# getterupper/PreWorld

Hardware: AMD Instinct MI355X
Metric: samples/sec (6-cam frame -> 200x200x16 occ) (higher is better)
Workload: dtype f32 as hi+lo f16 (3 MFMA per product block, f32 accumulate)

## Files before the change

preworld_amd/csrc/pw_forecast.hip:

```cpp
#include "pw_h2.h"

typedef float f32x16 __attribute__((ext_vector_type(16)));

namespace {
constexpr int C = 32;
constexpr int HID = 128;
constexpr int W1P = 4 * 4 * 64 * 4;
constexpr int W2P = 4 * 4 * 64 * 4;
}

__device__ __forceinline__ int row_of(int r, int h) { return (r & 3) + 8 * (r >> 2) + 4 * h; }

__device__ __forceinline__ float softplus_t20(float x) {
  const float t = __builtin_amdgcn_exp2f(-fabsf(x) * 1.44269504088896341f);
  return fmaf(__builtin_amdgcn_logf(1.f + t), 0.693147180559945309f, fmaxf(x, 0.f));
}

__global__ void __launch_bounds__(256)
k_forecast_prologue(const float* __restrict__ ego, int ego_dim, const float* __restrict__ w0,
                    const float* __restrict__ b0, const float* __restrict__ w2,
                    const float* __restrict__ b2, const float* __restrict__ w4,
                    const float* __restrict__ b4, const float* __restrict__ fw1,
                    const float* __restrict__ fb1, float* __restrict__ ego_feat,
                    float* __restrict__ c1, float* __restrict__ c1p) {
  __shared__ float h1[256], h2[256], e[C];
  const int t = threadIdx.x, s = blockIdx.x;
  const float* x = ego + (size_t)s * ego_dim;
  float acc = b0[t];
  for (int i = 0; i < ego_dim; ++i) acc += x[i] * w0[t * ego_dim + i];
  h1[t] = fmaxf(acc, 0.f);
  __syncthreads();
  acc = b2[t];
  for (int i = 0; i < 256; ++i) acc += h1[i] * w2[t * 256 + i];
  h2[t] = fmaxf(acc, 0.f);
  __syncthreads();
  if (t < C) {
    acc = b4[t];
    for (int i = 0; i < 256; ++i) acc += h2[i] * w4[t * 256 + i];
    e[t] = acc;
    ego_feat[(size_t)s * C + t] = acc;
  }
  __syncthreads();
  if (t < HID) {
    acc = fb1[t];
    for (int i = 0; i < C; ++i) acc += e[i] * fw1[t * 2 * C + C + i];
    c1[(size_t)s * HID + t] = acc;
    const int tile = t >> 5, row = t & 31;
    const int h = (row >> 2) & 1, r = (row & 3) + 4 * (row >> 3);
    c1p[(size_t)s * HID + h * 64 + tile * 16 + r] = acc;
  }
}

__global__ void k_forecast_pack(const float* __restrict__ fw1, const float* __restrict__ fw2,
                                float* __restrict__ w1p, float* __restrict__ w2p) {
  int idx = blockIdx.x * blockDim.x + threadIdx.x;
  if (idx >= W1P) return;
  int e = idx & 3, lane = (idx >> 2) & 63, q = (idx >> 8) & 3, t = idx >> 10;
  int i = lane & 31, h = lane >> 5;
  int k = row_of(4 * q + e, h);
  w1p[idx] = fw1[(size_t)(t * 32 + i) * (2 * C) + k];
  w2p[idx] = fw2[(size_t)i * HID + t * 32 + k];
}

__global__ void __launch_bounds__(256, 4)
k_forecast(const float* __restrict__ v0, long long n_vox_per_sample, int n_samples,
           const float* __restrict__ w1p, const float* __restrict__ w2p,
           const float* __restrict__ c1p, const float* __restrict__ fb2, int n_steps,
           float* __restrict__ states ) {
  extern __shared__ __attribute__((aligned(16))) float lds[];
  float* l_w1 = lds;
  float* l_w2 = lds + W1P;
  const int tid = threadIdx.x, lane = tid & 63, wave = tid >> 6;
  const int h = lane >> 5, j = lane & 31;
  for (int k = tid; k < W1P / 4; k += 256) {
    reinterpret_cast<float4*>(l_w1)[k] = reinterpret_cast<const float4*>(w1p)[k];
    reinterpret_cast<float4*>(l_w2)[k] = reinterpret_cast<const float4*>(w2p)[k];
  }
  __syncthreads();

  const long long n_total = n_vox_per_sample * n_samples;
  const long long n_tiles = (n_total + 31) / 32;
  float b2r[16];
#pragma unroll
  for (int s = 0; s < 16; ++s) b2r[s] = fb2[row_of(s, h)];

  for (long long tile = (long long)blockIdx.x * 4 + wave; tile < n_tiles;
       tile += (long long)gridDim.x * 4) {
    const long long m0 = tile * 32;
    long long m = m0 + j;
    const bool valid = m < n_total;
    if (!valid) m = n_total - 1;
    const int sample = (int)(m / n_vox_per_sample);
    const float* c1s = c1p + (size_t)sample * HID + h * 64;
    float v[16];
    const float* src = v0 + (size_t)m * C + 4 * h;
#pragma unroll
    for (int q = 0; q < 4; ++q) {
      float4 t4 = *reinterpret_cast<const float4*>(src + 8 * q);
      v[4 * q + 0] = t4.x; v[4 * q + 1] = t4.y; v[4 * q + 2] = t4.z; v[4 * q + 3] = t4.w;
    }
    for (int step = 0; step < n_steps; ++step) {
      f32x16 o;
#pragma unroll
      for (int s = 0; s < 16; ++s) o[s] = b2r[s];
#pragma unroll 1
      for (int t = 0; t < 4; ++t) {
        f32x16 hid;
#pragma unroll
        for (int q = 0; q < 4; ++q) {
          const float4 c4 = *reinterpret_cast<const float4*>(c1s + t * 16 + q * 4);
          hid[4 * q + 0] = c4.x; hid[4 * q + 1] = c4.y; hid[4 * q + 2] = c4.z; hid[4 * q + 3] = c4.w;
        }
#pragma unroll
        for (int sq = 0; sq < 4; ++sq) {
          const float4 a4 = *reinterpret_cast<const float4*>(l_w1 + ((t * 4 + sq) * 64 + lane) * 4);
          const float av[4] = {a4.x, a4.y, a4.z, a4.w};
#pragma unroll
          for (int e = 0; e < 4; ++e)
            hid = __builtin_amdgcn_mfma_f32_32x32x2f32(av[e], v[4 * sq + e], hid, 0, 0, 0);
        }
#pragma unroll
        for (int r = 0; r < 16; ++r) hid[r] = softplus_t20(hid[r]);
#pragma unroll
        for (int rq = 0; rq < 4; ++rq) {
          const float4 a4 = *reinterpret_cast<const float4*>(l_w2 + ((t * 4 + rq) * 64 + lane) * 4);
          const float av[4] = {a4.x, a4.y, a4.z, a4.w};
#pragma unroll
          for (int e = 0; e < 4; ++e)
            o = __builtin_amdgcn_mfma_f32_32x32x2f32(av[e], hid[4 * rq + e], o, 0, 0, 0);
        }
      }
#pragma unroll
      for (int s = 0; s < 16; ++s) v[s] = o[s] + v[s];
      if (valid) {
        float* dst = states + ((size_t)step * n_total + m) * C + 4 * h;
#pragma unroll
        for (int q = 0; q < 4; ++q)
          *reinterpret_cast<float4*>(dst + 8 * q) =
              make_float4(v[4 * q + 0], v[4 * q + 1], v[4 * q + 2], v[4 * q + 3]);
      }
    }
  }
}

PW_API int pw_forecast_pack(const float* fusion_w1, const float* fusion_w2, float* w1p, float* w2p,
                            void* stream) {
  PW_CHECK_ARG(fusion_w1 && fusion_w2 && w1p && w2p, "pw_forecast_pack: null pointer");
  hipLaunchKernelGGL(k_forecast_pack, dim3(W1P / 256), dim3(256), 0, pw_stream(stream), fusion_w1,
                     fusion_w2, w1p, w2p);
  PW_CHECK_LAUNCH();
  return PW_OK;
}

PW_API int pw_forecast_prologue(const float* ego, int n_samples, int ego_dim, const float* plan_w0,
                                const float* plan_b0, const float* plan_w2, const float* plan_b2,
                                const float* plan_w4, const float* plan_b4, const float* fusion_w1,
                                const float* fusion_b1, float* ego_feat, float* c1, float* c1p,
                                void* stream) {
  PW_CHECK_ARG(ego && plan_w0 && plan_b0 && plan_w2 && plan_b2 && plan_w4 && plan_b4 && fusion_w1 &&
                   fusion_b1 && ego_feat && c1 && c1p,
               "pw_forecast_prologue: null pointer");
  PW_CHECK_ARG(n_samples > 0 && ego_dim > 0, "pw_forecast_prologue: bad sizes");
  hipLaunchKernelGGL(k_forecast_prologue, dim3(n_samples), dim3(256), 0, pw_stream(stream), ego,
                     ego_dim, plan_w0, plan_b0, plan_w2, plan_b2, plan_w4, plan_b4, fusion_w1,
                     fusion_b1, ego_feat, c1, c1p);
  PW_CHECK_LAUNCH();
  return PW_OK;
}

PW_API int pw_forecast_steps(const float* v0, int64_t n_vox_per_sample, int n_samples,
                             const float* w1p, const float* w2p, const float* c1p,
                             const float* fusion_b2, int n_steps, float* states, void* stream) {
  PW_CHECK_ARG(v0 && w1p && w2p && c1p && fusion_b2 && states, "pw_forecast_steps: null pointer");
  PW_CHECK_ARG(n_vox_per_sample > 0 && n_samples > 0 && n_steps > 0, "pw_forecast_steps: bad sizes");
  PW_CHECK_ARG((((uintptr_t)v0 | (uintptr_t)states | (uintptr_t)w1p | (uintptr_t)w2p) & 15) == 0,
               "pw_forecast_steps: pointers must be 16-B aligned");
  const size_t lds_bytes = (size_t)(W1P + W2P) * 4;
  long long n_tiles = (n_vox_per_sample * n_samples + 31) / 32;
  long long want = (n_tiles + 3) / 4;
  unsigned nb = (unsigned)(want < 1280 ? want : 1280);
  hipLaunchKernelGGL(k_forecast, dim3(nb), dim3(256), lds_bytes, pw_stream(stream), v0,
                     (long long)n_vox_per_sample, n_samples, w1p, w2p, c1p, fusion_b2, n_steps,
                     states);
  pw_note_kernel("k_forecast");
  PW_CHECK_LAUNCH();
  return PW_OK;
}

typedef _Float16 fh8 __attribute__((ext_vector_type(8)));
typedef _Float16 fh4 __attribute__((ext_vector_type(4)));
typedef float fv4 __attribute__((ext_vector_type(4)));
constexpr int WH2 = 4 * 2 * 2 * 64 * 4;

__device__ __forceinline__ void split8(const float* x, fh8& hi, fh8& lo) {
  const float v[8] = {x[0], x[1], x[2], x[3], x[4], x[5], x[6], x[7]};
  h8 a, b;
  h2_split8(v, a, b);
  hi = __builtin_bit_cast(fh8, a);
  lo = __builtin_bit_cast(fh8, b);
}

__device__ __forceinline__ void split8_bounded(const float* x, fh8& hi, fh8& lo) {
  typedef _Float16 sh2 __attribute__((ext_vector_type(2)));
  typedef float sf2 __attribute__((ext_vector_type(2)));
  unsigned hp[4], lp[4];
#pragma unroll
  for (int p = 0; p < 4; ++p) {
    const sf2 v = {x[2 * p], x[2 * p + 1]};
    hp[p] = __builtin_bit_cast(unsigned, __builtin_convertvector(v, sh2));
    unsigned l;
    asm("v_fma_mixlo_f16 %0, %1, -1.0, %2 op_sel:[0,0,0] op_sel_hi:[1,0,0]" : "=v"(l) : "v"(hp[p]), "v"(v[0]));
    asm("v_fma_mixhi_f16 %0, %1, -1.0, %2 op_sel:[1,0,0] op_sel_hi:[1,0,0]" : "+v"(l) : "v"(hp[p]), "v"(v[1]));
    lp[p] = l;
  }
  typedef unsigned su4 __attribute__((ext_vector_type(4)));
  hi = __builtin_bit_cast(fh8, su4{hp[0], hp[1], hp[2], hp[3]});
  lo = __builtin_bit_cast(fh8, su4{lp[0], lp[1], lp[2], lp[3]});
}

__device__ __forceinline__ float softplus_scaled(float zs, float kexp, float kln) {
  const float t = __builtin_amdgcn_exp2f(-fabsf(zs) * kexp);
  return fmaf(__builtin_amdgcn_logf(1.f + t), kln, fmaxf(zs, 0.f));
}

__global__ void __launch_bounds__(256, 2)
k_forecast_h2(const float* __restrict__ v0, long long n_vox_per_sample, int n_samples, const float* __restrict__ w1p,
              const float* __restrict__ w2p, float inv1, float inv2, const float* __restrict__ c1p,
              const float* __restrict__ fb2, int n_steps, float* __restrict__ states, int v0_h2, int out_h2,
              const int* __restrict__ v0_rng, int* __restrict__ st_rng, float w1_l1max) {
#ifdef PW_X_SKIP_FC
  return;
#endif
  extern __shared__ __attribute__((aligned(16))) float lds[];
  float* l_w1 = lds;
  float* l_w2 = lds + WH2;
  float* l_c1 = lds + 2 * WH2;
  const int tid = threadIdx.x, lane = tid & 63, wave = tid >> 6;
  const int h = lane >> 5, j = lane & 31;
  const int e0 = v0_h2 ? rng_exp(v0_rng) : 0;
  const int eu = rng_exp(st_rng);
  unsigned cmb = 0u;
  for (int k = lane; k < n_samples * HID; k += 64) cmb = max(cmb, rng_absbits(c1p[k]));
  for (int k = tid; k < WH2 / 4; k += 256) {
    reinterpret_cast<float4*>(l_w1)[k] = reinterpret_cast<const float4*>(w1p)[k];
    reinterpret_cast<float4*>(l_w2)[k] = reinterpret_cast<const float4*>(w2p)[k];
  }
  int eh;
  {
    const float cmax = __uint_as_float(wave_umax(cmb));
    const float zb = fmaf(w1_l1max, rng_pow2(16 + eu), cmax + 1.f);
    int ex;
    (void)frexpf(zb, &ex);
    eh = __builtin_amdgcn_readfirstlane(ex) - 15;
    eh = eh < -100 ? -100 : (eh > 100 ? 100 : eh);
  }
  for (int k = tid; k < n_samples * HID; k += 256) l_c1[k] = c1p[k] * rng_pow2(-eh);
  __syncthreads();
  auto uni_f = [](float x) { return __int_as_float(__builtin_amdgcn_readfirstlane(__float_as_int(x))); };
  const float k_in = uni_f(rng_pow2(e0 - eu));
  const float k1 = uni_f(inv1 * rng_pow2(eu - eh));
  const float k2 = uni_f(inv2 * rng_pow2(eh - eu));
  const float kexp = uni_f(1.44269504088896341f * rng_pow2(eh)), kln = uni_f(0.693147180559945309f * rng_pow2(-eh));
  const float k_out = uni_f(rng_pow2(eu));
  const long long n_total = n_vox_per_sample * n_samples;
  const long long n_tiles = (n_total + 31) / 32;
  float b2r[16];
#pragma unroll
  for (int s = 0; s < 16; ++s) b2r[s] = fb2[row_of(s, h)] * rng_pow2(-eu);
  float amax = 0.f;
  unsigned lastbits = 0u;
  const char* a1 = reinterpret_cast<const char*>(l_w1) + lane * 16;
  const char* a2 = reinterpret_cast<const char*>(l_w2) + lane * 16;

  constexpr int NU = 2;
  const long long n_pairs = (n_tiles + NU - 1) / NU;
  for (long long pair = (long long)blockIdx.x * 4 + wave; pair < n_pairs; pair += (long long)gridDim.x * 4) {
    long long m[NU];
    bool valid[NU];
    const float* c1s[NU];
    float v[NU][16];
    fh8 vh[NU][2], vl[NU][2];
#pragma unroll
    for (int u = 0; u < NU; ++u) {
      m[u] = (pair * NU + u) * 32 + j;
      valid[u] = m[u] < n_total;
      if (!valid[u]) m[u] = n_total - 1;
      const int sample = (int)(m[u] / n_vox_per_sample);
      c1s[u] = l_c1 + (size_t)sample * HID + h * 64;
      if (v0_h2) {
        const char* src = reinterpret_cast<const char*>(v0 + (size_t)m[u] * C) + 8 * h;
#pragma unroll
        for (int q = 0; q < 4; ++q) {
          const int off = (4 * (q & 1) + 2 * (q >> 1)) * 16;
          const fh4 hi4 = *reinterpret_cast<const fh4*>(src + off), lo4 = *reinterpret_cast<const fh4*>(src + off + 16);
#pragma unroll
          for (int e = 0; e < 4; ++e) v[u][4 * q + e] = ((float)hi4[e] + (float)lo4[e]) * k_in;
        }
      } else {
        const float* src = v0 + (size_t)m[u] * C + 4 * h;
#pragma unroll
        for (int q = 0; q < 4; ++q) {
          float4 t4 = *reinterpret_cast<const float4*>(src + 8 * q);
          v[u][4 * q + 0] = t4.x * k_in; v[u][4 * q + 1] = t4.y * k_in; v[u][4 * q + 2] = t4.z * k_in; v[u][4 * q + 3] = t4.w * k_in;
        }
      }
      split8(v[u], vh[u][0], vl[u][0]);
      split8(v[u] + 8, vh[u][1], vl[u][1]);
    }
    for (int step = 0; step < n_steps; ++step) {
      f32x16 o[NU];
#pragma unroll
      for (int u = 0; u < NU; ++u)
#pragma unroll
        for (int s = 0; s < 16; ++s) o[u][s] = 0.f;
#pragma unroll 1
      for (int t = 0; t < 4; ++t) {
        f32x16 hid[NU];
#pragma unroll
        for (int u = 0; u < NU; ++u)
#pragma unroll
          for (int s = 0; s < 16; ++s) hid[u][s] = 0.f;
#pragma unroll
        for (int ks = 0; ks < 2; ++ks) {
          const fh8 wh = __builtin_bit_cast(fh8, *reinterpret_cast<const fv4*>(a1 + ((t * 2 + ks) * 2 + 0) * 1024));
          const fh8 wl = __builtin_bit_cast(fh8, *reinterpret_cast<const fv4*>(a1 + ((t * 2 + ks) * 2 + 1) * 1024));
#pragma unroll
          for (int u = 0; u < NU; ++u) {
            hid[u] = __builtin_amdgcn_mfma_f32_32x32x16_f16(wh, vh[u][ks], hid[u], 0, 0, 0);
            hid[u] = __builtin_amdgcn_mfma_f32_32x32x16_f16(wl, vh[u][ks], hid[u], 0, 0, 0);
            hid[u] = __builtin_amdgcn_mfma_f32_32x32x16_f16(wh, vl[u][ks], hid[u], 0, 0, 0);
          }
        }
        fh8 hh[NU][2], hl[NU][2];
#pragma unroll
        for (int u = 0; u < NU; ++u) {
          float hs[16];
#pragma unroll
          for (int q = 0; q < 4; ++q) {
            const float4 c4 = *reinterpret_cast<const float4*>(c1s[u] + t * 16 + q * 4);
            hs[4 * q + 0] = softplus_scaled(fmaf(hid[u][4 * q + 0], k1, c4.x), kexp, kln);
            hs[4 * q + 1] = softplus_scaled(fmaf(hid[u][4 * q + 1], k1, c4.y), kexp, kln);
            hs[4 * q + 2] = softplus_scaled(fmaf(hid[u][4 * q + 2], k1, c4.z), kexp, kln);
            hs[4 * q + 3] = softplus_scaled(fmaf(hid[u][4 * q + 3], k1, c4.w), kexp, kln);
          }
#ifdef PW_X_FC_OLD_SPLIT
          split8(hs, hh[u][0], hl[u][0]);
          split8(hs + 8, hh[u][1], hl[u][1]);
#else
          split8_bounded(hs, hh[u][0], hl[u][0]);
          split8_bounded(hs + 8, hh[u][1], hl[u][1]);
#endif
        }
#pragma unroll
        for (int kb = 0; kb < 2; ++kb) {
          const fh8 wh = __builtin_bit_cast(fh8, *reinterpret_cast<const fv4*>(a2 + ((t * 2 + kb) * 2 + 0) * 1024));
          const fh8 wl = __builtin_bit_cast(fh8, *reinterpret_cast<const fv4*>(a2 + ((t * 2 + kb) * 2 + 1) * 1024));
#pragma unroll
          for (int u = 0; u < NU; ++u) {
            o[u] = __builtin_amdgcn_mfma_f32_32x32x16_f16(wh, hh[u][kb], o[u], 0, 0, 0);
            o[u] = __builtin_amdgcn_mfma_f32_32x32x16_f16(wl, hh[u][kb], o[u], 0, 0, 0);
            o[u] = __builtin_amdgcn_mfma_f32_32x32x16_f16(wh, hl[u][kb], o[u], 0, 0, 0);
          }
        }
      }
#pragma unroll
      for (int u = 0; u < NU; ++u) {
#pragma unroll
        for (int s = 0; s < 16; ++s) v[u][s] = fmaf(o[u][s], k2, b2r[s]) + v[u][s];
        split8(v[u], vh[u][0], vl[u][0]);
        split8(v[u] + 8, vh[u][1], vl[u][1]);
        if (valid[u]) {
#pragma unroll
          for (int s = 0; s < 16; ++s) amax = fmaxf(amax, fabsf(v[u][s]));
          if (out_h2) {
            fh4 hi4[4], lo4[4];
#pragma unroll
            for (int q = 0; q < 4; ++q)
#pragma unroll
              for (int e = 0; e < 4; ++e) {
                hi4[q][e] = vh[u][q >> 1][4 * (q & 1) + e];
                lo4[q][e] = vl[u][q >> 1][4 * (q & 1) + e];
              }
            char* dst = reinterpret_cast<char*>(states + ((size_t)step * n_total + m[u]) * C);
#pragma unroll
            for (int qq = 0; qq < 2; ++qq)
#pragma unroll
              for (int p = 0; p < 2; ++p) {
                typedef unsigned fu2 __attribute__((ext_vector_type(2)));
                typedef unsigned fu4 __attribute__((ext_vector_type(4)));
                const fu2 a = __builtin_bit_cast(fu2, p ? lo4[qq] : hi4[qq]), b = __builtin_bit_cast(fu2, p ? lo4[qq + 2] : hi4[qq + 2]);
                const auto s0 = __builtin_amdgcn_permlane32_swap(a[0], b[0], false, false);
                const auto s1 = __builtin_amdgcn_permlane32_swap(a[1], b[1], false, false);
                fu4 slot;
                slot[0] = s0[0]; slot[1] = s1[0]; slot[2] = s0[1]; slot[3] = s1[1];
                *reinterpret_cast<fu4*>(dst + (4 * qq + 2 * h + p) * 16) = slot;
              }
          } else {
            float* dst = states + ((size_t)step * n_total + m[u]) * C + 4 * h;
#pragma unroll
            for (int q = 0; q < 4; ++q)
              *reinterpret_cast<float4*>(dst + 8 * q) = make_float4(v[u][4 * q + 0] * k_out, v[u][4 * q + 1] * k_out, v[u][4 * q + 2] * k_out,
                                                                    v[u][4 * q + 3] * k_out);
          }
        }
      }
    }
#pragma unroll
    for (int u = 0; u < NU; ++u)
      if (valid[u]) {
#pragma unroll
        for (int s = 0; s < 16; ++s) lastbits = max(lastbits, rng_absbits(v[u][s]));
      }
  }
  rng_note(st_rng, max(__float_as_uint(amax), lastbits), eu);
}

PW_API int pw_forecast_steps_h2(const float* v0, int64_t n_vox_per_sample, int n_samples, const float* w1p,
                                const float* w2p, float inv1, float inv2, const float* c1p, const float* fusion_b2,
                                int n_steps, float* states, int v0_h2, int out_h2, const int32_t* v0_rng, int32_t* states_rng,
                                float w1_l1max, void* stream) {
  PW_CHECK_ARG(v0 && w1p && w2p && c1p && fusion_b2 && states, "pw_forecast_steps_h2: null pointer");
  PW_CHECK_ARG(n_vox_per_sample > 0 && n_samples > 0 && n_samples <= 64 && n_steps > 0, "pw_forecast_steps_h2: bad sizes (<= 64 samples)");
  PW_CHECK_ARG(w1_l1max >= 0.f, "pw_forecast_steps_h2: w1_l1max = max row L1 norm of fusion_head.0.weight[:, :32]");
  PW_CHECK_ARG((((uintptr_t)v0 | (uintptr_t)states | (uintptr_t)w1p | (uintptr_t)w2p) & 15) == 0,
               "pw_forecast_steps_h2: pointers must be 16-B aligned");
  const size_t lds_bytes = (size_t)2 * WH2 * 4 + (size_t)n_samples * HID * 4;
  long long n_tiles = (n_vox_per_sample * n_samples + 31) / 32;
  long long want = ((n_tiles + 1) / 2 + 3) / 4;
  unsigned nb = (unsigned)(want < 512 ? want : 512);
  hipLaunchKernelGGL(k_forecast_h2, dim3(nb), dim3(256), lds_bytes, pw_stream(stream), v0, (long long)n_vox_per_sample,
                     n_samples, w1p, w2p, inv1, inv2, c1p, fusion_b2, n_steps, states, v0_h2, out_h2, v0_rng, states_rng, w1_l1max);
  pw_note_kernel("k_forecast_h2");
  PW_CHECK_LAUNCH();
  return PW_OK;
}

constexpr int ATTR_TILES = 6;
constexpr int ATTR_WP = ATTR_TILES * 4 * 64 * 4;
constexpr int ATTR_GC = 24;

__global__ void __launch_bounds__(256, 3)
k_attr_mlp(const float* __restrict__ v0, long long n_vox, const float* __restrict__ w1p,
           const float* __restrict__ w2p, const float* __restrict__ b1p ,
           const float* __restrict__ b2 , int final_softplus, float* __restrict__ out) {
  extern __shared__ __attribute__((aligned(16))) float lds[];
  float* l_w1 = lds;
  float* l_w2 = lds + ATTR_WP;
  const int tid = threadIdx.x, lane = tid & 63, wave = tid >> 6;
  const int h = lane >> 5, j = lane & 31;
  for (int k = tid; k < ATTR_WP / 4; k += 256) {
    reinterpret_cast<float4*>(l_w1)[k] = reinterpret_cast<const float4*>(w1p)[k];
    reinterpret_cast<float4*>(l_w2)[k] = reinterpret_cast<const float4*>(w2p)[k];
  }
  __syncthreads();
  float b2r[16];
#pragma unroll
  for (int s = 0; s < 16; ++s) b2r[s] = b2[row_of(s, h)];
  const float* b1s = b1p + h * (ATTR_TILES * 16);
  const long long n_tiles = (n_vox + 31) / 32;
  for (long long tile = (long long)blockIdx.x * 4 + wave; tile < n_tiles;
       tile += (long long)gridDim.x * 4) {
    long long m = tile * 32 + j;
    const bool valid = m < n_vox;
    if (!valid) m = n_vox - 1;
    float v[16];
    const float* src = v0 + (size_t)m * C + 4 * h;
#pragma unroll
    for (int q = 0; q < 4; ++q) {
      float4 t4 = *reinterpret_cast<const float4*>(src + 8 * q);
      v[4 * q + 0] = t4.x; v[4 * q + 1] = t4.y; v[4 * q + 2] = t4.z; v[4 * q + 3] = t4.w;
    }
    f32x16 o;
#pragma unroll
    for (int s = 0; s < 16; ++s) o[s] = b2r[s];
#pragma unroll 1
    for (int t = 0; t < ATTR_TILES; ++t) {
      f32x16 hid;
#pragma unroll
      for (int q = 0; q < 4; ++q) {
        const float4 c4 = *reinterpret_cast<const float4*>(b1s + t * 16 + q * 4);
        hid[4 * q + 0] = c4.x; hid[4 * q + 1] = c4.y; hid[4 * q + 2] = c4.z; hid[4 * q + 3] = c4.w;
      }
#pragma unroll
      for (int sq = 0; sq < 4; ++sq) {
        const float4 a4 = *reinterpret_cast<const float4*>(l_w1 + ((t * 4 + sq) * 64 + lane) * 4);
        const float av[4] = {a4.x, a4.y, a4.z, a4.w};
#pragma unroll
        for (int e = 0; e < 4; ++e)
          hid = __builtin_amdgcn_mfma_f32_32x32x2f32(av[e], v[4 * sq + e], hid, 0, 0, 0);
      }
#pragma unroll
      for (int r = 0; r < 16; ++r) hid[r] = softplus_t20(hid[r]);
#pragma unroll
      for (int rq = 0; rq < 4; ++rq) {
        const float4 a4 = *reinterpret_cast<const float4*>(l_w2 + ((t * 4 + rq) * 64 + lane) * 4);
        const float av[4] = {a4.x, a4.y, a4.z, a4.w};
#pragma unroll
        for (int e = 0; e < 4; ++e)
          o = __builtin_amdgcn_mfma_f32_32x32x2f32(av[e], hid[4 * rq + e], o, 0, 0, 0);
      }
    }
    if (final_softplus && h == 0) {
      o[0] = softplus_t20(o[0]);
      o[1] = softplus_t20(o[1]);
    }
    if (valid) {
      float* dst = out + (size_t)m * ATTR_GC + 4 * h;
#pragma unroll
      for (int q = 0; q < 3; ++q)
        *reinterpret_cast<float4*>(dst + 8 * q) =
            make_float4(o[4 * q + 0], o[4 * q + 1], o[4 * q + 2], o[4 * q + 3]);
    }
  }
}

PW_API int pw_attr_mlp(const float* v0, int64_t n_vox, const float* w1p, const float* w2p,
                       const float* b1p, const float* b2, int final_softplus, float* out,
                       void* stream) {
  PW_CHECK_ARG(v0 && w1p && w2p && b1p && b2 && out && n_vox > 0, "pw_attr_mlp: bad arguments");
  PW_CHECK_ARG((((uintptr_t)v0 | (uintptr_t)out | (uintptr_t)w1p | (uintptr_t)w2p) & 15) == 0,
               "pw_attr_mlp: pointers must be 16-B aligned");
  const size_t lds_bytes = (size_t)ATTR_WP * 2 * 4;
  long long want = ((n_vox + 31) / 32 + 3) / 4;
  unsigned nb = (unsigned)(want < 768 ? want : 768);
  hipLaunchKernelGGL(k_attr_mlp, dim3(nb), dim3(256), lds_bytes, pw_stream(stream), v0,
                     (long long)n_vox, w1p, w2p, b1p, b2, final_softplus, out);
  PW_CHECK_LAUNCH();
  return PW_OK;
}

__global__ void k_softplus(const float* __restrict__ x, float* __restrict__ y, long long n) {
  long long i = (long long)blockIdx.x * blockDim.x + threadIdx.x;
  if (i < n) y[i] = softplus_t20(x[i]);
}

PW_API int pw_softplus(const float* x, float* y, int64_t n, void* stream) {
  PW_CHECK_ARG(x && y && n > 0, "pw_softplus: bad arguments");
  hipLaunchKernelGGL(k_softplus, dim3((unsigned)pw_cdiv(n, 256)), dim3(256), 0, pw_stream(stream), x,
                     y, (long long)n);
  PW_CHECK_LAUNCH();
  return PW_OK;
}

__global__ void __launch_bounds__(256)
k_global_avgpool(const float* __restrict__ x, int64_t n_vox, int C, float* __restrict__ y) {
  const float* xb = x + (size_t)blockIdx.x * n_vox * C;
  for (int c = threadIdx.x; c < C; c += blockDim.x) {
    float s = 0.f;
    for (int64_t v = 0; v < n_vox; ++v) s += xb[v * C + c];
    y[(size_t)blockIdx.x * C + c] = s / (float)n_vox;
  }
}

__global__ void __launch_bounds__(256)
k_linear_act(const float* __restrict__ x, const float* __restrict__ w, const float* __restrict__ b,
             float* __restrict__ y, int n_in, int n_out, int act) {
  const float* xr = x + (size_t)blockIdx.x * n_in;
  for (int o = threadIdx.x; o < n_out; o += blockDim.x) {
    float acc = b ? b[o] : 0.f;
    const float* wo = w + (size_t)o * n_in;
    for (int k = 0; k < n_in; ++k) acc += xr[k] * wo[k];
    if (act == 1) acc = fmaxf(acc, 0.f);
    else if (act == 2) acc = softplus_t20(acc);
    y[(size_t)blockIdx.x * n_out + o] = acc;
  }
}

PW_API int pw_global_avgpool_ndhwc(const float* x, int B, int64_t n_vox, int C, float* y, void* stream) {
  PW_CHECK_ARG(x && y && B > 0 && n_vox > 0 && C > 0, "pw_global_avgpool_ndhwc: bad arguments");
  hipLaunchKernelGGL(k_global_avgpool, dim3((unsigned)B), dim3(256), 0, pw_stream(stream), x, n_vox, C, y);
  PW_CHECK_LAUNCH();
  return PW_OK;
}

PW_API int pw_linear_act(const float* x, const float* w, const float* b, float* y, int rows, int n_in,
                         int n_out, int act, void* stream) {
  PW_CHECK_ARG(x && w && y && rows > 0 && n_in > 0 && n_out > 0, "pw_linear_act: bad arguments");
  PW_CHECK_ARG(act >= 0 && act <= 2, "pw_linear_act: act must be 0 (none), 1 (ReLU) or 2 (Softplus)");
  hipLaunchKernelGGL(k_linear_act, dim3((unsigned)rows), dim3(256), 0, pw_stream(stream), x, w, b, y, n_in,
                     n_out, act);
  PW_CHECK_LAUNCH();
  return PW_OK;
}
```

Before: 396.1.

## Software-pipeline forecast MLP across hidden chunks with one tile per wave

Restructures the forecast kernel so each wave processes one 32-voxel tile instead of two, and software-pipelines the two GEMMs. The first-layer MFMAs for the next hidden chunk are interleaved with the softplus and split of the current chunk and the second-layer MFMAs. Scheduling barriers keep the interleave in place. Register use drops, so launch bounds rise to 3 blocks per CU and the grid cap goes up to 768. This trades two-tile ILP for software pipelining plus higher occupancy, at the risk of register spills or weaker MFMA overlap.

```diff
diff --git a/preworld_amd/csrc/pw_forecast.hip b/preworld_amd/csrc/pw_forecast.hip
--- a/preworld_amd/csrc/pw_forecast.hip
+++ b/preworld_amd/csrc/pw_forecast.hip
@@ -223,7 +223,13 @@
   return fmaf(__builtin_amdgcn_logf(1.f + t), kln, fmaxf(zs, 0.f));
 }
 
-__global__ void __launch_bounds__(256, 2)
+__device__ __forceinline__ void fc_mfma(const char* aw, int t, int n, const fh8 (&xh)[2], const fh8 (&xl)[2], f32x16& acc) {
+  const int kb = n / 3, p = n % 3;
+  const fh8 w = __builtin_bit_cast(fh8, *reinterpret_cast<const fv4*>(aw + ((t * 2 + kb) * 2 + (p == 1 ? 1 : 0)) * 1024));
+  acc = __builtin_amdgcn_mfma_f32_32x32x16_f16(w, p == 2 ? xl[kb] : xh[kb], acc, 0, 0, 0);
+}
+
+__global__ void __launch_bounds__(256, 3)
 k_forecast_h2(const float* __restrict__ v0, long long n_vox_per_sample, int n_samples, const float* __restrict__ w1p,
               const float* __restrict__ w2p, float inv1, float inv2, const float* __restrict__ c1p,
               const float* __restrict__ fb2, int n_steps, float* __restrict__ states, int v0_h2, int out_h2,
@@ -272,145 +278,121 @@
   const char* a1 = reinterpret_cast<const char*>(l_w1) + lane * 16;
   const char* a2 = reinterpret_cast<const char*>(l_w2) + lane * 16;
 
-  constexpr int NU = 2;
-  const long long n_pairs = (n_tiles + NU - 1) / NU;
-  for (long long pair = (long long)blockIdx.x * 4 + wave; pair < n_pairs; pair += (long long)gridDim.x * 4) {
-    long long m[NU];
-    bool valid[NU];
-    const float* c1s[NU];
-    float v[NU][16];
-    fh8 vh[NU][2], vl[NU][2];
-#pragma unroll
-    for (int u = 0; u < NU; ++u) {
-      m[u] = (pair * NU + u) * 32 + j;
-      valid[u] = m[u] < n_total;
-      if (!valid[u]) m[u] = n_total - 1;
-      const int sample = (int)(m[u] / n_vox_per_sample);
-      c1s[u] = l_c1 + (size_t)sample * HID + h * 64;
-      if (v0_h2) {
-        const char* src = reinterpret_cast<const char*>(v0 + (size_t)m[u] * C) + 8 * h;
-#pragma unroll
-        for (int q = 0; q < 4; ++q) {
-          const int off = (4 * (q & 1) + 2 * (q >> 1)) * 16;
-          const fh4 hi4 = *reinterpret_cast<const fh4*>(src + off), lo4 = *reinterpret_cast<const fh4*>(src + off + 16);
-#pragma unroll
-          for (int e = 0; e < 4; ++e) v[u][4 * q + e] = ((float)hi4[e] + (float)lo4[e]) * k_in;
+  for (long long tile = (long long)blockIdx.x * 4 + wave; tile < n_tiles; tile += (long long)gridDim.x * 4) {
+    long long m = tile * 32 + j;
+    const bool valid = m < n_total;
+    if (!valid) m = n_total - 1;
+    const int sample = (int)(m / n_vox_per_sample);
+    const float* c1s = l_c1 + (size_t)sample * HID + h * 64;
+    float v[16];
+    fh8 vh[2], vl[2];
+    if (v0_h2) {
+      const char* src = reinterpret_cast<const char*>(v0 + (size_t)m * C) + 8 * h;
+#pragma unroll
+      for (int q = 0; q < 4; ++q) {
+        const int off = (4 * (q & 1) + 2 * (q >> 1)) * 16;
+        const fh4 hi4 = *reinterpret_cast<const fh4*>(src + off), lo4 = *reinterpret_cast<const fh4*>(src + off + 16);
+#pragma unroll
+        for (int e = 0; e < 4; ++e) v[4 * q + e] = ((float)hi4[e] + (float)lo4[e]) * k_in;
+      }
+    } else {
+      const float* src = v0 + (size_t)m * C + 4 * h;
+#pragma unroll
+      for (int q = 0; q < 4; ++q) {
+        float4 t4 = *reinterpret_cast<const float4*>(src + 8 * q);
+        v[4 * q + 0] = t4.x * k_in; v[4 * q + 1] = t4.y * k_in; v[4 * q + 2] = t4.z * k_in; v[4 * q + 3] = t4.w * k_in;
+      }
+    }
+    split8(v, vh[0], vl[0]);
+    split8(v + 8, vh[1], vl[1]);
+    f32x16 hid[2];
+    auto gemm1_first = [&]() {
+#pragma unroll
+      for (int s = 0; s < 16; ++s) hid[0][s] = 0.f;
+#pragma unroll
+      for (int n = 0; n < 6; ++n) fc_mfma(a1, 0, n, vh, vl, hid[0]);
+    };
+    gemm1_first();
+    for (int step = 0; step < n_steps; ++step) {
+      f32x16 o;
+#pragma unroll
+      for (int s = 0; s < 16; ++s) o[s] = 0.f;
+#pragma unroll
+      for (int t = 0; t < 4; ++t) {
+        const int cur = t & 1, nxt = cur ^ 1;
+        if (t < 3) {
+#pragma unroll
+          for (int s = 0; s < 16; ++s) hid[nxt][s] = 0.f;
         }
-      } else {
-        const float* src = v0 + (size_t)m[u] * C + 4 * h;
-#pragma unroll
-        for (int q = 0; q < 4; ++q) {
-          float4 t4 = *reinterpret_cast<const float4*>(src + 8 * q);
-          v[u][4 * q + 0] = t4.x * k_in; v[u][4 * q + 1] = t4.y * k_in; v[u][4 * q + 2] = t4.z * k_in; v[u][4 * q + 3] = t4.w * k_in;
+        float hs[16];
+        fh8 hh[2], hl[2];
+#pragma unroll
+        for (int c = 0; c < 4; ++c) {
+          const float4 c4 = *reinterpret_cast<const float4*>(c1s + t * 16 + c * 4);
+          hs[4 * c + 0] = softplus_scaled(fmaf(hid[cur][4 * c + 0], k1, c4.x), kexp, kln);
+          hs[4 * c + 1] = softplus_scaled(fmaf(hid[cur][4 * c + 1], k1, c4.y), kexp, kln);
+          hs[4 * c + 2] = softplus_scaled(fmaf(hid[cur][4 * c + 2], k1, c4.z), kexp, kln);
+          hs[4 * c + 3] = softplus_scaled(fmaf(hid[cur][4 * c + 3], k1, c4.w), kexp, kln);
+          if (c & 1) split8_bounded(hs + 8 * (c >> 1), hh[c >> 1], hl[c >> 1]);
+          if (t < 3) {
+#pragma unroll
+            for (int n = (c * 3) / 2; n < ((c + 1) * 3) / 2; ++n) fc_mfma(a1, t + 1, n, vh, vl, hid[nxt]);
+          }
+          if (c == 2) {
+#pragma unroll
+            for (int n = 0; n < 3; ++n) fc_mfma(a2, t, n, hh, hl, o);
+          }
+          __builtin_amdgcn_sched_barrier(0x180);
         }
-      }
-      split8(v[u], vh[u][0], vl[u][0]);
-      split8(v[u] + 8, vh[u][1], vl[u][1]);
-    }
-    for (int step = 0; step < n_steps; ++step) {
-      f32x16 o[NU];
-#pragma unroll
-      for (int u = 0; u < NU; ++u)
-#pragma unroll
-        for (int s = 0; s < 16; ++s) o[u][s] = 0.f;
-#pragma unroll 1
-      for (int t = 0; t < 4; ++t) {
-        f32x16 hid[NU];
-#pragma unroll
-        for (int u = 0; u < NU; ++u)
-#pragma unroll
-          for (int s = 0; s < 16; ++s) hid[u][s] = 0.f;
-#pragma unroll
-        for (int ks = 0; ks < 2; ++ks) {
-          const fh8 wh = __builtin_bit_cast(fh8, *reinterpret_cast<const fv4*>(a1 + ((t * 2 + ks) * 2 + 0) * 1024));
-          const fh8 wl = __builtin_bit_cast(fh8, *reinterpret_cast<const fv4*>(a1 + ((t * 2 + ks) * 2 + 1) * 1024));
-#pragma unroll
-          for (int u = 0; u < NU; ++u) {
-            hid[u] = __builtin_amdgcn_mfma_f32_32x32x16_f16(wh, vh[u][ks], hid[u], 0, 0, 0);
-            hid[u] = __builtin_amdgcn_mfma_f32_32x32x16_f16(wl, vh[u][ks], hid[u], 0, 0, 0);
-            hid[u] = __builtin_amdgcn_mfma_f32_32x32x16_f16(wh, vl[u][ks], hid[u], 0, 0, 0);
-          }
+#pragma unroll
+        for (int n = 3; n < 6; ++n) fc_mfma(a2, t, n, hh, hl, o);
+      }
+#pragma unroll
+      for (int s = 0; s < 16; ++s) v[s] = fmaf(o[s], k2, b2r[s]) + v[s];
+      split8(v, vh[0], vl[0]);
+      split8(v + 8, vh[1], vl[1]);
+      if (valid) {
+#pragma unroll
+        for (int s = 0; s < 16; ++s) amax = fmaxf(amax, fabsf(v[s]));
+      }
+      if (step + 1 < n_steps) gemm1_first();
+      if (valid) {
+        if (out_h2) {
+          fh4 hi4[4], lo4[4];
+#pragma unroll
+          for (int q = 0; q < 4; ++q)
+#pragma unroll
+            for (int e = 0; e < 4; ++e) {
+              hi4[q][e] = vh[q >> 1][4 * (q & 1) + e];
+              lo4[q][e] = vl[q >> 1][4 * (q & 1) + e];
+            }
+          char* dst = reinterpret_cast<char*>(states + ((size_t)step * n_total + m) * C);
+#pragma unroll
+          for (int qq = 0; qq < 2; ++qq)
+#pragma unroll
+            for (int p = 0; p < 2; ++p) {
+              typedef unsigned fu2 __attribute__((ext_vector_type(2)));
+              typedef unsigned fu4 __attribute__((ext_vector_type(4)));
+              const fu2 a = __builtin_bit_cast(fu2, p ? lo4[qq] : hi4[qq]), b = __builtin_bit_cast(fu2, p ? lo4[qq + 2] : hi4[qq + 2]);
+              const auto s0 = __builtin_amdgcn_permlane32_swap(a[0], b[0], false, false);
+              const auto s1 = __builtin_amdgcn_permlane32_swap(a[1], b[1], false, false);
+              fu4 slot;
+              slot[0] = s0[0]; slot[1] = s1[0]; slot[2] = s0[1]; slot[3] = s1[1];
+              *reinterpret_cast<fu4*>(dst + (4 * qq + 2 * h + p) * 16) = slot;
+            }
+        } else {
+          float* dst = states + ((size_t)step * n_total + m) * C + 4 * h;
+#pragma unroll
+          for (int q = 0; q < 4; ++q)
+            *reinterpret_cast<float4*>(dst + 8 * q) = make_float4(v[4 * q + 0] * k_out, v[4 * q + 1] * k_out, v[4 * q + 2] * k_out,
+                                                                  v[4 * q + 3] * k_out);
         }
-        fh8 hh[NU][2], hl[NU][2];
-#pragma unroll
-        for (int u = 0; u < NU; ++u) {
-          float hs[16];
-#pragma unroll
-          for (int q = 0; q < 4; ++q) {
-            const float4 c4 = *reinterpret_cast<const float4*>(c1s[u] + t * 16 + q * 4);
-            hs[4 * q + 0] = softplus_scaled(fmaf(hid[u][4 * q + 0], k1, c4.x), kexp, kln);
-            hs[4 * q + 1] = softplus_scaled(fmaf(hid[u][4 * q + 1], k1, c4.y), kexp, kln);
-            hs[4 * q + 2] = softplus_scaled(fmaf(hid[u][4 * q + 2], k1, c4.z), kexp, kln);
-            hs[4 * q + 3] = softplus_scaled(fmaf(hid[u][4 * q + 3], k1, c4.w), kexp, kln);
-          }
-#ifdef PW_X_FC_OLD_SPLIT
-          split8(hs, hh[u][0], hl[u][0]);
-          split8(hs + 8, hh[u][1], hl[u][1]);
-#else
-          split8_bounded(hs, hh[u][0], hl[u][0]);
-          split8_bounded(hs + 8, hh[u][1], hl[u][1]);
-#endif
-        }
-#pragma unroll
-        for (int kb = 0; kb < 2; ++kb) {
-          const fh8 wh = __builtin_bit_cast(fh8, *reinterpret_cast<const fv4*>(a2 + ((t * 2 + kb) * 2 + 0) * 1024));
-          const fh8 wl = __builtin_bit_cast(fh8, *reinterpret_cast<const fv4*>(a2 + ((t * 2 + kb) * 2 + 1) * 1024));
-#pragma unroll
-          for (int u = 0; u < NU; ++u) {
-            o[u] = __builtin_amdgcn_mfma_f32_32x32x16_f16(wh, hh[u][kb], o[u], 0, 0, 0);
-            o[u] = __builtin_amdgcn_mfma_f32_32x32x16_f16(wl, hh[u][kb], o[u], 0, 0, 0);
-            o[u] = __builtin_amdgcn_mfma_f32_32x32x16_f16(wh, hl[u][kb], o[u], 0, 0, 0);
-          }
-        }
-      }
-#pragma unroll
-      for (int u = 0; u < NU; ++u) {
-#pragma unroll
-        for (int s = 0; s < 16; ++s) v[u][s] = fmaf(o[u][s], k2, b2r[s]) + v[u][s];
-        split8(v[u], vh[u][0], vl[u][0]);
-        split8(v[u] + 8, vh[u][1], vl[u][1]);
-        if (valid[u]) {
-#pragma unroll
-          for (int s = 0; s < 16; ++s) amax = fmaxf(amax, fabsf(v[u][s]));
-          if (out_h2) {
-            fh4 hi4[4], lo4[4];
-#pragma unroll
-            for (int q = 0; q < 4; ++q)
-#pragma unroll
-              for (int e = 0; e < 4; ++e) {
-                hi4[q][e] = vh[u][q >> 1][4 * (q & 1) + e];
-                lo4[q][e] = vl[u][q >> 1][4 * (q & 1) + e];
-              }
-            char* dst = reinterpret_cast<char*>(states + ((size_t)step * n_total + m[u]) * C);
-#pragma unroll
-            for (int qq = 0; qq < 2; ++qq)
-#pragma unroll
-              for (int p = 0; p < 2; ++p) {
-                typedef unsigned fu2 __attribute__((ext_vector_type(2)));
-                typedef unsigned fu4 __attribute__((ext_vector_type(4)));
-                const fu2 a = __builtin_bit_cast(fu2, p ? lo4[qq] : hi4[qq]), b = __builtin_bit_cast(fu2, p ? lo4[qq + 2] : hi4[qq + 2]);
-                const auto s0 = __builtin_amdgcn_permlane32_swap(a[0], b[0], false, false);
-                const auto s1 = __builtin_amdgcn_permlane32_swap(a[1], b[1], false, false);
-                fu4 slot;
-                slot[0] = s0[0]; slot[1] = s1[0]; slot[2] = s0[1]; slot[3] = s1[1];
-                *reinterpret_cast<fu4*>(dst + (4 * qq + 2 * h + p) * 16) = slot;
-              }
-          } else {
-            float* dst = states + ((size_t)step * n_total + m[u]) * C + 4 * h;
-#pragma unroll
-            for (int q = 0; q < 4; ++q)
-              *reinterpret_cast<float4*>(dst + 8 * q) = make_float4(v[u][4 * q + 0] * k_out, v[u][4 * q + 1] * k_out, v[u][4 * q + 2] * k_out,
-                                                                    v[u][4 * q + 3] * k_out);
-          }
-        }
-      }
-    }
-#pragma unroll
-    for (int u = 0; u < NU; ++u)
-      if (valid[u]) {
-#pragma unroll
-        for (int s = 0; s < 16; ++s) lastbits = max(lastbits, rng_absbits(v[u][s]));
-      }
+      }
+    }
+    if (valid) {
+#pragma unroll
+      for (int s = 0; s < 16; ++s) lastbits = max(lastbits, rng_absbits(v[s]));
+    }
   }
   rng_note(st_rng, max(__float_as_uint(amax), lastbits), eu);
 }
@@ -426,8 +408,8 @@
                "pw_forecast_steps_h2: pointers must be 16-B aligned");
   const size_t lds_bytes = (size_t)2 * WH2 * 4 + (size_t)n_samples * HID * 4;
   long long n_tiles = (n_vox_per_sample * n_samples + 31) / 32;
-  long long want = ((n_tiles + 1) / 2 + 3) / 4;
-  unsigned nb = (unsigned)(want < 512 ? want : 512);
+  long long want = (n_tiles + 3) / 4;
+  unsigned nb = (unsigned)(want < 768 ? want : 768);
   hipLaunchKernelGGL(k_forecast_h2, dim3(nb), dim3(256), lds_bytes, pw_stream(stream), v0, (long long)n_vox_per_sample,
                      n_samples, w1p, w2p, inv1, inv2, c1p, fusion_b2, n_steps, states, v0_h2, out_h2, v0_rng, states_rng, w1_l1max);
   pw_note_kernel("k_forecast_h2");
```

Result: no change. 398.3 (median of 2 runs) (+0.5%).
